# refresh-bio/kmer-db

Hardware: AMD Instinct MI355X
Metric: all2all k-mer pair-comparisons/sec (higher is better)
Workload: dtype u32

## Files before the change

### kmer-db_amd/csrc/a2a_blocks.hip

```cpp
#include "device_common.h"
#include "engine_internal.h"

#include "prim.h"

#include <algorithm>
#include <chrono>
#include <cmath>
#include <cstdio>
#include <cstdlib>
#include <cstring>
#include <functional>
#include <memory>
#include <string>

enum : uint32_t {
    KCTR_CHUNKS = 0,
    KCTR_POOL_OVERFLOW,
    KCTR_PAIR_OVERFLOW,
    KCTR_NWIDE,
    KCTR_LIST_OVERFLOW,
    KCTR_RAW = 5,
    KCTR_RECORDS = 6,
    KCTR_RECORDS_HI = 7,
    KCTR_SLOW = 8,
// ... 295 lines not shown
template <class PV> __device__ __forceinline__ void rowtab_finish(const RowTab& R, const PV& pv, uint32_t lane) {
    lds_sync();
    for (uint32_t X = lane; X < R.n; X += WAVE) {
        const uint32_t e = R.end[X];
        if (e) pool_cold(pv)->chunk_fill[(e - 1u) >> CH_SHIFT] = CH_REC - (e - R.pos[X]);
    }
}
template <bool ROWS, class PV>
__device__ __forceinline__ void rec_emit(WaveArena& A, const PV& pv, const RowTab& R, bool on, uint32_t X, unsigned long long rows, unsigned long long cols,
                                         uint32_t w, uint32_t stream, uint32_t lane, unsigned long long lt_mask) {
    if constexpr (ROWS) row_emit(A, pv, R, on, X, rows, cols, w, stream, lane, lt_mask);
    else wide_emit(A, pv, on, rows, cols, w, stream, lane, lt_mask);
}
__device__ __forceinline__ void rec_store_diag(const PoolView& pv, uint32_t slot, unsigned long long rows, uint32_t w) {
    const uint32_t ch = slot >> CH_SHIFT, r = slot & (CH_REC - 1u);
    ((unsigned long long*)(pv.rec + ((size_t)ch << (CH_SHIFT + 4))))[r] = rows;
    pv.recw[slot] = w;
}

__global__ void call_prologue_kernel(uint32_t* __restrict__ state, uint32_t n_state, uint32_t* __restrict__ chunk_fill, uint32_t* __restrict__ chunk_key,
                                     uint32_t pool_cap, unsigned char* __restrict__ touched, uint32_t n_touched) {
    const uint32_t i = blockIdx.x * blockDim.x + threadIdx.x;
    if (i < n_state) state[i] = 0u;
    if (i < pool_cap) { chunk_fill[i] = 0u; chunk_key[i] = 0xFFFFFFFFu; }
    if (i < n_touched) touched[i] = 0;
}

struct K0Params {
    const uint2* k0in;
    const uint32_t* bitrel;
    const uint64_t* blkbase;
    const uint64_t* bits;
    const uint32_t* perm;
    uint32_t P;
    uint32_t short_ids;
    BlockMap bm;
    unsigned long long* p0_mask;
    uint32_t* p0_info;
    uint32_t* pair_ofs;
    uint16_t* pair_blk;
    unsigned long long* pair_mask;
    uint32_t* pair_cursor;
    uint32_t n_regions, region_cap, spill_cap;
    uint32_t* counters;
};

constexpr int K0_RELW = 8;
constexpr int K0_SINGLE_PASS = 1;
template <bool LONG>
__global__ __launch_bounds__(256) void k0_decode_kernel(const K0Params q) {
    const uint32_t t = blockIdx.x * blockDim.x + threadIdx.x;
    const uint32_t lane = threadIdx.x & 63u;
    uint32_t i = 0;
    bool live;
    if (q.perm) {
        live = t < q.P;
        if (live) i = q.perm[t];
    } else {
        __shared__ uint32_t bins[64];
        __shared__ uint16_t order[256];
        if (threadIdx.x < 64) bins[threadIdx.x] = 0;
        __syncthreads();
        const uint2 kt = t < q.P ? q.k0in[t] : make_uint2(0u, 0u);
        const uint32_t tl = kmdb_k0_l(kt), tbits = kmdb_k0_bits(kt);
        uint32_t key = 0;
        if (t < q.P && tl > 1 && !kmdb_long_node(tl, tbits, q.short_ids)) {
            key = 1u + (tbits - (tl - 1u));
            key = key > 63u ? 63u : key;
        }
        atomicAdd(&bins[63u - key], 1u);
        __syncthreads();
        if (threadIdx.x < 64) {
            const uint32_t c = bins[threadIdx.x];
            bins[threadIdx.x] = wave_incl_scan(c, threadIdx.x) - c;
        }
        __syncthreads();
        order[atomicAdd(&bins[63u - key], 1u)] = (uint16_t)threadIdx.x;
        __syncthreads();
        i = blockIdx.x * blockDim.x + order[threadIdx.x];
        live = i < q.P;
    }
    const BlockMap bm = q.bm;
    const uint2 km = live ? q.k0in[i] : make_uint2(0u, 0u);
    const uint32_t l = kmdb_k0_l(km), last = kmdb_k0_last(km), nbits = kmdb_k0_bits(km);
    if (!q.perm && kmdb_long_node(l, nbits, q.short_ids)) live = false;
    using Cursor = RunCursor32<LONG ? 16 : 6, LONG>;
    uint32_t npairs = 0, blk0 = 0, need = 0, span = 0, bit0 = 0;
    unsigned long long mask0 = 0, m1 = 0, m2 = 0;
    bool second_pass = false, from_words = false;
    uint64_t pos = 0;
    unsigned long long rel_w[K0_RELW];
    uint32_t rel_i[K0_RELW], rel_n = 0;
#pragma unroll
    for (int e = 0; e < K0_RELW; ++e) { rel_w[e] = 0; rel_i[e] = 0; }
    auto rel_push = [&](uint32_t idx, unsigned long long w) {
#pragma unroll
        for (int e = 0; e < K0_RELW; ++e) if (rel_n == (uint32_t)e) { rel_w[e] = w; rel_i[e] = idx; }
        ++rel_n;
    };
    auto rel_blocks = [&](bool write, uint32_t id0, uint32_t o) -> uint32_t {
        const unsigned long long wm = bm.width == 64 ? ~0ull : (1ull << bm.width) - 1ull;
        uint32_t curblk = 0xFFFFFFFFu, cnt = 0;
        unsigned long long cacc = 0;
        auto flushb = [&]() {
            if (curblk == 0xFFFFFFFFu) return;
            if (write) { if (cnt == 0) mask0 = cacc; else { q.pair_blk[o] = (uint16_t)curblk; q.pair_mask[o] = cacc; ++o; } }
            ++cnt;
        };
#pragma unroll
        for (int e = 0; e < K0_RELW; ++e) {
            if ((uint32_t)e < rel_n) {
                const uint32_t base = id0 + 64u * rel_i[e];
                const unsigned long long word = rel_w[e];
                const uint32_t b = bm.blk(base);
                uint32_t bit = bm.bit(base, b), sh = 0;
#pragma unroll
                for (uint32_t part = 0; part < 3; ++part) {
                    if (sh < 64u) {
                        const unsigned long long m = ((word >> sh) << bit) & wm;
                        if (m) {
                            if (b + part != curblk) { flushb(); curblk = b + part; cacc = 0; }
                            cacc |= m;
                        }
                        sh += bm.width - bit; bit = 0;
                    }
                }
            }
        }
        flushb();
        return cnt;
    };
    if (live && l == 1) {
        blk0 = bm.blk(last); mask0 = 1ull << bm.bit(last, blk0); npairs = 1;
    } else if (live && l) {
        pos = q.blkbase[i >> 8] + q.bitrel[i];
        unsigned long long R = 1ull;
        {
            Cursor c(q.bits, pos);
            uint32_t rem = l - 1;
            uint32_t wk = 0;
            unsigned long long acc = 1ull;
            auto add = [&](uint32_t s0, uint32_t cnt) {
                while (cnt) {
                    const uint32_t k = s0 >> 6, o = s0 & 63u;
                    const uint32_t take = cnt < 64u - o ? cnt : 64u - o;
                    if (k != wk) { rel_push(wk, acc); wk = k; acc = 0; }
                    acc |= (take == 64u ? ~0ull : ((1ull << take) - 1ull)) << o;
                    s0 += take; cnt -= take;
                }
            };
            while (rem) {
                uint32_t z, v;
                c.step(rem, z, v);
                if (z) {
                    if (LONG) add(span + 1u, z);
                    else if (span + z < 64u) R |= ((2ull << (z - 1)) - 1ull) << (span + 1);
                    span += z; rem -= z;
                }
                if (v) {
                    span += v; --rem;
                    if (LONG) add(span, 1u);
                    else if (span < 64u) R |= 1ull << span;
                }
            }
            if (LONG) { if (span < 64u) R = acc; else rel_push(wk, acc); }
        }
        const uint32_t id0 = last - span;
        blk0 = bm.blk(id0);
        bit0 = bm.bit(id0, blk0);
        const unsigned long long wm = bm.width == 64 ? ~0ull : (1ull << bm.width) - 1ull;
// ... 2657 lines not shown
    const size_t W = node_cap / 64u, NB = b.NB;
    DEV_ALLOC(b.l2_cursors, 2 * L2_SUB * 16);
    DEV_ALLOC(b.l2_bitmap, NB * W);
    DEV_ALLOC(b.l2_rank, NB * W);
    DEV_ALLOC(b.l2_len, NB);
    DEV_ALLOC(b.l2_loff, NB + 2);
    DEV_ALLOC(b.l2_ent_g, (size_t)ent_cap);
    DEV_ALLOC(b.l2_ent_blk, (size_t)ent_cap);
    DEV_ALLOC(b.l2_ent_mask, (size_t)ent_cap);
    DEV_ALLOC(b.l2_list_mask, (size_t)ent_cap);
    DEV_ALLOC(b.l2_list_w, (size_t)ent_cap);
    DEV_ALLOC(b.l2_node_w, (size_t)node_cap);
    b.l2_node_cap = node_cap; b.l2_ent_cap = ent_cap;
    return 0;
}

struct Launched { uint32_t raw = 0, rowjobs = 0, k2jobs = 0; };
inline uint32_t with_slack(uint32_t v) { return v + v / 8u + 1024u; }
int stage_done(hipStream_t s, const char* name) {
    if (!kmdb_sync_debug()) return 0;
    const hipError_t e = hipStreamSynchronize(s);
    fprintf(stderr, "[kmdb] stage %-14s %s\n", name, e == hipSuccess ? "ok" : hipGetErrorString(e));
    return e == hipSuccess ? 0 : kmdb_set_error(std::string("stage ") + name + ": " + hipGetErrorString(e));
}
void a2a_prologue(BlocksState& b, hipStream_t st, bool decode) {
    const uint32_t pool_cap = (uint32_t)b.pool_cap;
    const uint32_t n_state = decode ? b.call_state_n_decode : b.call_state_n, n_touched = decode && b.tile_touched ? b.n_states + 1u : 0u;
    hipLaunchKernelGGL(call_prologue_kernel, dim3((std::max(std::max(n_state, pool_cap), n_touched) + 255u) / 256u), dim3(256), 0, st, b.call_state.get(), n_state,
                       b.chunk_fill.get(), b.chunk_key.get(), pool_cap, b.tile_touched.get(), n_touched);
}
int a2a_decode(kmdb_db* db, BlocksState& b, hipStream_t st) {
    const uint32_t P = (uint32_t)db->P;
    K0Params q{};
    q.k0in = db->k0in; q.bitrel = db->bitrel; q.blkbase = db->blkbase; q.bits = db->bits; q.perm = nullptr; q.P = P; q.short_ids = db->short_max_ids;
    q.bm = BlockMap{db->width, (uint32_t)((1ull << 32) / db->width) + 1u};
    q.p0_mask = b.p0_mask; q.p0_info = b.p0_info; q.pair_ofs = b.pair_ofs; q.pair_blk = b.pair_blk; q.pair_mask = b.pair_mask;
    uint32_t nreg = 1;
    while (nreg < KMDB_PAIR_REGIONS && (uint64_t)nreg * 16384 < P) nreg <<= 1;
    q.pair_cursor = b.pair_cursor; q.n_regions = nreg; q.region_cap = (uint32_t)(b.pair_cap * 3 / 4 / nreg);
    q.spill_cap = (uint32_t)(b.pair_cap - (uint64_t)q.region_cap * nreg); q.counters = b.counters;
    hipLaunchKernelGGL((k0_decode_kernel<false>), dim3((P + 255) / 256), dim3(256), 0, st, q);
    if (db->n_long) {
        q.perm = db->long_nodes; q.P = db->n_long;
        hipLaunchKernelGGL((k0_decode_kernel<true>), dim3((db->n_long + 255) / 256), dim3(256), 0, st, q);
    }
    HIP_TRY(hipGetLastError());
    return 0;
}
int a2a_narrow_emit(kmdb_db* db, BlocksState& b, uint32_t* M, uint32_t emit_lo, uint32_t emit_hi, hipStream_t st) {
    NParams q{};
    q.nl = db->nl; q.parent = db->parent; q.w = db->w; q.dflag = db->dflag; q.seg_anc = db->nseg_anc; q.seg_anc_n = db->nseg_anc_n;
    q.p0_mask = b.p0_mask; q.p0_info = b.p0_info; q.pair_ofs = b.pair_ofs; q.pair_blk = b.pair_blk; q.pair_mask = b.pair_mask;
    q.fn_mask = b.fn_mask; q.fn_blk = b.fn_blk; q.widebits = b.widebits; q.wide_base = b.wide_base; q.wide_slice_cnt = b.wide_slice_cnt;
    q.P = (uint32_t)db->P; q.nseg_nodes = db->nseg_nodes; q.n_segs = db->n_nsegs; q.chain_cap = db->chain_cap;
    q.emit_lo = emit_lo; q.emit_hi = emit_hi; q.tbits = b.dense_narrow ? 0u : arena_table_bits(b.g_rows); q.n_keys = b.g_rows;
    q.all_wide = b.dense_narrow ? 1u : 0u;
    q.pool = pool_view(b, b.dense_narrow);
    q.band_xlo = b.g_xlo; q.band_xhi = b.g_xhi; q.band_sbase = b.g_sbase;
    const size_t wave_lds = k1n_wave_bytes(q.chain_cap, q.tbits, q.n_keys, b.row_mode ? b.g_rows : 0u);
    const uint32_t waves = (uint32_t)std::max<size_t>(1, std::min<size_t>(K1N_WAVES, (144u << 10) / wave_lds));
    const size_t lds = wave_lds * waves;
    q.M = M; q.N = (uint32_t)db->N; q.bwidth = db->width; q.touched = touched_view(b); q.direct_ctr = b.direct_ctr;
    q.dmask = b.dmask; q.dwx = b.dwx; q.slice_cnt = b.slice_cnt;
    const K1nPick pick = b.emit_band ? k1n_band_pick(b.k1n_mode, b.row_mode) : k1n_pick(b.k1n_mode, b.knobs.k1n_minw, b.row_mode);
    HIP_TRY(hipFuncSetAttribute((const void*)pick.fn, hipFuncAttributeMaxDynamicSharedMemorySize, (int)lds));
    const dim3 grid((q.n_segs + waves - 1) / waves), block(WAVE * waves);
    if (!b.have_counts && kmdb_verbose())
        fprintf(stderr, "[kmdb] narrow kernel: %u slices, %zu B of LDS per wave, %u per workgroup, instantiation %s\n", q.n_segs, wave_lds, waves, pick.name);
    hipLaunchKernelGGL(pick.fn, grid, block, lds, st, q);
    HIP_TRY(hipGetLastError());
    return 0;
}
int a2a_slice_apply(kmdb_db* db, BlocksState& b, uint32_t* M, hipStream_t st, hipStream_t s2) {
    HIP_TRY(hipEventRecord(db->ev_side[0], st));
// ... 498 lines not shown
```

### kmer-db_amd/csrc/engine_state.h

```cpp
#pragma once
#include "kmdb_amd.h"
#include "kmdb_internal.h"

#include <thread>
#include "engine_internal.h"
#include "dev_mem.h"

#include <hip/hip_runtime.h>

#include <cstdint>
#include <memory>
#include <string>
#include <utility>
#include <vector>

struct Segment { uint32_t first, end; };

struct BlocksState;
struct BlocksStateDelete { void operator()(BlocksState* b) const; };

struct kmdb_db {
    int device = 0;
    uint64_t N = 0, P = 0;
    uint32_t kmer_length = 0;
    DevBuf<uint2> k0in;
    DevBuf<uint32_t> bitrel;
    DevBuf<uint64_t> blkbase;
    DevBuf<uint64_t> bits;
    uint64_t n_bit_words = 0;
    uint32_t short_max_ids = 48;
    DevBuf<uint32_t> nl;
    DevBuf<int32_t> parent;
    DevBuf<uint32_t> w;
    DevBuf<uint16_t> dflag;
    DevBuf<uint32_t> sub_end;
    DevBuf<uint32_t> long_nodes;
    uint32_t n_long = 0;
    uint32_t nseg_nodes = 2048;
    uint32_t n_nsegs = 0;
    DevBuf<uint32_t> nseg_anc;
    DevBuf<uint32_t> nseg_anc_n;
    uint32_t chain_cap = 8;
    uint32_t max_depth = 0, max_n = 0;
    DevBuf<unsigned long long> list_sets;
    uint32_t list_sets_nb = 0;
    bool list_sets_tried = false;
    DevBuf<uint32_t> rl_ofs;
    DevBuf<uint32_t> rl_runs;
    DevBuf<uint4> rl_node;
    bool rl_tried = false;
    bool chain_ok = false;
    uint32_t width = 64;
    std::unique_ptr<BlocksState, BlocksStateDelete> blocks;
    uint64_t blocks_bytes_counted = 0;
    bool last_call_sized = false;
    std::vector<std::pair<void*, size_t>> staging;
    std::vector<std::pair<void*, size_t>> staging_kept;
    std::thread staging_thread;
    bool one_shot = false;
    bool v1_ready = false;
    DevBuf<uint4> meta;
    DevBuf<uint64_t> bitpos;
    DevBuf<uint32_t> ck_ofs;
    DevBuf<uint64_t> ck_bit;
    DevBuf<uint32_t> ck_id;
    DevBuf<uint32_t> wprefix;
    DevBuf<Segment> segs;
    uint32_t n_segs = 0;
    DevBuf<void> v1_scan_tmp;
    size_t v1_scan_tmp_bytes = 0;
// ... 25 lines not shown
    uint64_t band_max_streams = 0;
    int band_emit_mode = -2;
    kmdb_all2all_rows_band_emit_stats be_stats{};
    uint64_t n_buckets = 0;
    DevBuf<uint64_t> bucket_offset;
    DevBuf<uint64_t> slots;
    DevBuf<uint32_t> pid2dfs;
    uint32_t qs_index = 0, qs_count = 0;
    hipStream_t stream = nullptr;
    hipStream_t stream2 = nullptr;
    DevEvent ev_side[2], ev[4];
    DevEvent ev_k[4];
    kmdb_stats stats{};
    kmdb_db2db_stats d2_stats{};
    kmdb_new2all_sparse_stats n2s_stats{};
    kmdb_sample_stats sample_stats{};
    kmdb_sample_stats d2_sample_stats{};
    kmdb_sample_stats n2a_sample_stats{};
    bool blocks_prepared = false;
    std::string fallback_reason;
};

constexpr uint32_t KMDB_MAX_STREAM_BITS = 1u << 24;
__host__ __device__ inline uint2 kmdb_k0_pack(uint32_t l, uint32_t last, uint32_t nbits) {
    uint2 r;
    r.x = l | ((nbits >> 12) << KMDB_ID_BITS); r.y = last | ((nbits & 0xFFFu) << KMDB_ID_BITS);
    return r;
}
__host__ __device__ inline uint32_t kmdb_k0_l(uint2 km) { return km.x & (KMDB_MAX_SAMPLES - 1u); }
__host__ __device__ inline uint32_t kmdb_k0_last(uint2 km) { return km.y & (KMDB_MAX_SAMPLES - 1u); }
__host__ __device__ inline uint32_t kmdb_k0_bits(uint2 km) { return ((km.x >> KMDB_ID_BITS) << 12) | (km.y >> KMDB_ID_BITS); }
constexpr uint32_t KMDB_SHORT_MAX_IDS = 48, KMDB_SHORT_MAX_BITS = 128;
__host__ __device__ inline bool kmdb_long_node(uint32_t l, uint32_t num_bits, uint32_t max_ids) { return l > max_ids || num_bits > KMDB_SHORT_MAX_BITS; }
constexpr int KMDB_CHAIN_MAX = 4096;

int kmdb_layout_upload(kmdb_db* db, const kmdb_db_view* v, int with_hashtables, const kmdb_kept_nodes* sel);
int kmdb_db_upload_planned(const kmdb_db_view* v, const kmdb_opts* opts, int with_hashtables, uint32_t shard_index, uint32_t shard_count, kmdb_shard_plan* plan,
                           kmdb_db** out);
int kmdb_db_upload_query_planned(const kmdb_db_view* v, const kmdb_opts* opts, uint32_t shard_index, uint32_t shard_count, kmdb_shard_plan* plan, kmdb_db** out);
int kmdb_db_upload_range_planned(const kmdb_db_view* v, const kmdb_opts* opts, uint32_t range_index, const kmdb_range_plan* plan, kmdb_db** out);

int kmdb_v1_run(kmdb_db* db, uint32_t* M, uint32_t seg_begin, uint32_t seg_end, uint32_t flags, hipStream_t st);

int kmdb_blocks_prepare(kmdb_db* db);
struct kmdb_band_desc { uint64_t row_lo, row_hi, cell_lo, cells; bool emit = false; };
int kmdb_blocks_run(kmdb_db* db, uint32_t* M, uint32_t emit_lo, uint32_t emit_hi, hipStream_t st, const kmdb_band_desc* band = nullptr);
std::string kmdb_blocks_band_refusal(const kmdb_db* db, const kmdb_band_geometry* g);
int kmdb_blocks_band_prepare(kmdb_db* db, const kmdb_band_geometry* g, uint64_t band_cells);
int kmdb_blocks_k1n_mode(const kmdb_db* db, bool band_state);
uint64_t kmdb_blocks_state_bytes(const kmdb_db* db, bool band_state);
struct kmdb_blocks_band_units { uint64_t jobs, jobs_run, runs, runs_run, slices, slices_run, tiles, tiles_run; };
struct kmdb_blocks_band_info { uint32_t key_bits, row_mode, l2_on, attempts, slices; uint64_t records, est_records; kmdb_blocks_band_units units; };
kmdb_blocks_band_info kmdb_blocks_band_last(const kmdb_db* db, bool band_state);
void kmdb_blocks_release(kmdb_db* db);
uint64_t kmdb_blocks_device_bytes(const kmdb_db* db);
int kmdb_blocks_ensure_prepared(kmdb_db* db);
int kmdb_blocks_stage_ms(kmdb_db* db, float ms[4]);
inline void kmdb_recount_bytes(kmdb_db* db, uint64_t& counted, uint64_t now) {
    db->stats.device_bytes = db->stats.device_bytes - counted + now;
    counted = now;
}
struct kmdb_blocks_counts { uint64_t records, direct; uint32_t wide, chunks, joined; };
kmdb_blocks_counts kmdb_blocks_last_counts(const kmdb_db* db);
const unsigned char* kmdb_blocks_tile_touched(const kmdb_db* db);
int kmdb_ensure_v1_arrays(kmdb_db* db);

// ... 2 lines not shown
```

### kmer-db_amd/csrc/kmdb_internal.h

```cpp
#pragma once
#include <cstddef>
#include <cstdint>
#include <functional>
#include <string>
#include <utility>
#include <vector>

int kmdb_set_error(const std::string& msg);

constexpr uint32_t KMDB_ABI_OLDEST_COMPATIBLE = 7, KMDB_ABI_THIS = 8;
inline bool kmdb_abi_compatible(uint32_t caller) { return caller >= KMDB_ABI_OLDEST_COMPATIBLE && caller <= KMDB_ABI_THIS; }

void kmdb_drop_pages(const std::vector<std::pair<void*, size_t>>& regions, unsigned threads);

struct kmdbh_db;
struct kmdbh_db_arrays {
    int64_t *num_kmers, *parent_id;
    uint32_t *num_samples, *num_local, *last_sample_id, *num_bits;
    uint64_t *data_offset, *data, *bucket_offset, *slots;
};
kmdbh_db* kmdbh_db_make(uint32_t kmer_length, double fraction, double start_fraction, int32_t alphabet, uint64_t kmers_count,
                        std::vector<std::string>&& names, std::vector<uint64_t>&& sample_kmers, uint64_t n_patterns, uint64_t n_data_words,
                        uint64_t n_buckets, uint64_t n_slots, kmdbh_db_arrays* arrays);

struct kmdb_db;
struct kmdb_layout_device_source {
    uint64_t n_patterns = 0, n_samples = 0;
    uint32_t kmer_length = 0;
    const long long* num_kmers = nullptr;
    const long long* parent_id = nullptr;
    const uint32_t* num_samples = nullptr;
    const uint32_t* num_local = nullptr;
    const uint32_t* last_sample_id = nullptr;
    const uint32_t* num_bits = nullptr;
    const unsigned long long* data_offset = nullptr;
    const uint64_t* data = nullptr;
    uint64_t n_data_words = 0;
    uint64_t n_buckets = 0, n_slots = 0;
    const uint64_t* bucket_offset = nullptr;
    const uint64_t* slots = nullptr;
    std::function<void()> tables_done, fields_done, streams_done;
    mutable double fields_ms = 0;
    double layout_ms = 0, prepare_ms = 0;
};
int kmdb_layout_from_device(kmdb_db* db, const kmdb_layout_device_source* src, int with_hashtables);
struct kmdb_opts;
int kmdb_db_from_device(kmdb_layout_device_source* src, const kmdb_opts* opts, int with_hashtables, kmdb_db** out);

using kmdb_device_lists_sink = std::function<int(const uint64_t* d_kmers, const uint64_t* off, size_t n, void* stream)>;
struct kmdb_opts;
int kmdb_minhash_device_lists(const char* who, const char* const* seqs, const size_t* seq_lens, size_t n_samples, uint32_t kmer_length, double fraction,
                              double start_fraction, int32_t alphabet, const kmdb_opts* opts, const kmdb_device_lists_sink& sink);

int kmdb_sorted_union_on_stream(const char* who, const uint64_t* a, uint64_t na, const uint64_t* b, uint64_t nb, uint64_t* out, uint64_t* n_out, void* stream,
                                uint64_t* scratch_bytes);

struct kmdb_db_view;
constexpr uint32_t KMDB_MAX_SHARDS = 4096;
struct kmdb_shard_plan {
    uint64_t P = 0;
    uint32_t n_shards = 0;
    std::vector<uint32_t*> w;
    std::vector<unsigned char*> mask;
    std::vector<uint64_t> kept;
    kmdb_shard_plan() = default;
    kmdb_shard_plan(const kmdb_shard_plan&) = delete;
    kmdb_shard_plan& operator=(const kmdb_shard_plan&) = delete;
    ~kmdb_shard_plan();
    void release_weights(uint32_t shard);
    bool keeps(uint32_t shard, uint64_t p) const { return (mask[shard >> 3][p] >> (shard & 7u)) & 1u; }
};
int kmdb_shard_plan_build(const kmdb_db_view* v, uint32_t n_shards, const std::vector<uint32_t>& shards, kmdb_shard_plan* plan);

void kmdb_query_shard_tables(const kmdb_db_view* v, uint32_t shard, uint32_t n_shards, uint64_t* n_buckets, uint64_t* n_slots);

template <class F>
inline void kmdb_for_bucket_runs(const uint64_t* kmers, size_t count, F&& fn) {
    for (size_t i = 0; i < count;) {
        const uint64_t b = kmers[i] >> 32;
        size_t e = i + 1;
// ... 44 lines not shown
```

### kmer-db_amd/csrc/layout.hip

```cpp
#include "device_common.h"
#include "engine_internal.h"

#include "prim.h"

#include <algorithm>
#include <atomic>
#include <chrono>
#include <cstdio>
#include <cstdlib>
#include <cstring>
#include <sys/mman.h>
#include <thread>

namespace {

struct U32toU64 { __host__ __device__ uint64_t operator()(uint32_t v) const { return v; } };

__global__ void lay_child_runs_kernel(const uint32_t* __restrict__ skeys, uint32_t P, uint32_t* __restrict__ start, uint32_t* __restrict__ cnt) {
    const uint32_t j = blockIdx.x * blockDim.x + threadIdx.x;
    if (j >= P) return;
    const uint32_t k = skeys[j];
    if (j == 0 || skeys[j - 1] != k) start[k] = j;
    if (j + 1 == P || skeys[j + 1] != k) cnt[k] = j + 1;
}
// ... 114 lines not shown
    if ((i & 255u) == 0) blkbase[i >> 8] = b;
    bitrel[i] = (uint32_t)(dstpos[i] - b);
}
__global__ void lay_copy_bits_kernel(const uint32_t* __restrict__ order, const uint64_t* __restrict__ srcpos, const uint64_t* __restrict__ dstpos,
                                     const uint2* __restrict__ k0in, const uint64_t* __restrict__ src, uint32_t P, unsigned long long* __restrict__ dst) {
    const uint32_t i = blockIdx.x * blockDim.x + threadIdx.x;
    if (i >= P) return;
    const uint32_t nb = kmdb_k0_bits(k0in[i]);
    if (!nb) return;
    uint64_t sp = srcpos[order[i]], dp = dstpos[i];
    for (uint32_t done = 0; done < nb; done += 64) {
        const uint32_t take = nb - done < 64u ? nb - done : 64u;
        const uint32_t ss = (uint32_t)(sp & 63u);
        uint64_t chunk = src[sp >> 6] << ss;
        if (ss && take > 64u - ss) chunk |= src[(sp >> 6) + 1] >> (64u - ss);
        if (take < 64u) chunk &= ~0ull << (64u - take);
        const uint32_t ds = (uint32_t)(dp & 63u);
        atomicOr(&dst[dp >> 6], (unsigned long long)(chunk >> ds));
        if (ds && take > 64u - ds) atomicOr(&dst[(dp >> 6) + 1], (unsigned long long)(chunk << (64u - ds)));
        sp += take; dp += take;
    }
}
struct LongNodePred {
    const uint2* k0in;
    uint32_t short_ids;
    __host__ __device__ bool operator()(uint32_t i) const { const uint2 km = k0in[i]; return kmdb_long_node(kmdb_k0_l(km), kmdb_k0_bits(km), short_ids); }
};
__global__ void lay_long_keys_kernel(const uint2* __restrict__ k0in, const uint32_t* __restrict__ idx, uint32_t n, uint32_t* __restrict__ keys) {
    const uint32_t t = blockIdx.x * blockDim.x + threadIdx.x;
    if (t >= n) return;
    const uint2 km = k0in[idx[t]];
    const uint32_t l = kmdb_k0_l(km);
    keys[t] = kmdb_k0_bits(km) - (l ? l - 1u : 0u);
}
__global__ void lay_seg_anc_kernel(const int32_t* __restrict__ parent, const uint16_t* __restrict__ dflag, uint32_t P, uint32_t nseg_nodes, uint32_t n_segs,
                                   uint32_t chain_cap, uint32_t* __restrict__ anc, uint32_t* __restrict__ anc_n) {
    const uint32_t s = blockIdx.x * blockDim.x + threadIdx.x;
    if (s >= n_segs) return;
    int32_t cur = parent[(size_t)s * nseg_nodes];
    uint32_t d = cur < 0 ? 0u : (uint32_t)(dflag[cur] & 0x7FFFu);
    if (d > chain_cap) d = 0;
    anc_n[s] = d;
    while (cur >= 0 && d) { anc[(size_t)s * chain_cap + (--d)] = (uint32_t)cur; cur = parent[cur]; }
}

struct HostRegion { void* p; size_t bytes; };
template <class T>
struct HostBuf {
    T* p = nullptr;
    size_t bytes = 0;
    explicit HostBuf(size_t n, bool zero = false) {
        (void)zero;
        bytes = (std::max<size_t>(n, 1) * sizeof(T) + 4095) & ~(size_t)4095;
        void* q = mmap(nullptr, bytes, PROT_READ | PROT_WRITE, MAP_PRIVATE | MAP_ANONYMOUS, -1, 0);
        p = q == MAP_FAILED ? nullptr : (T*)q;
    }
    ~HostBuf() { reset(); }
    void reset() { if (p) (void)munmap(p, bytes); p = nullptr; }
    HostRegion release() { HostRegion r{p, bytes}; p = nullptr; return r; }
    T& operator[](size_t i) { return p[i]; }
    HostBuf(const HostBuf&) = delete;
    HostBuf& operator=(const HostBuf&) = delete;
};

struct LayPhase {
    const bool verbose = getenv("KMDB_VERBOSE") != nullptr;
// ... 413 lines not shown
    if (in.streams_done) in.streams_done();
    phase("device: stream re-pack");

    db->max_n = hs.max_n; db->max_depth = hs.max_depth;
    db->chain_ok = hs.max_depth <= (uint32_t)KMDB_CHAIN_MAX;
    db->chain_cap = std::min<uint32_t>(KMDB_CHAIN_MAX, std::max<uint32_t>(8, (hs.max_depth + 7) / 8 * 8));
    db->nseg_nodes = 2048;
    if (const char* e = getenv("KMDB_NSEG")) if (*e) db->nseg_nodes = (uint32_t)std::max<uint64_t>(64, strtoull(e, nullptr, 10) / 64 * 64);
    db->n_nsegs = (uint32_t)((P + db->nseg_nodes - 1) / db->nseg_nodes);
    DEV_ALLOC(db->nseg_anc, std::max<size_t>((size_t)db->n_nsegs * db->chain_cap, 1));
    DEV_ALLOC(db->nseg_anc_n, std::max<size_t>(db->n_nsegs, 1));
    if (db->n_nsegs)
        hipLaunchKernelGGL(lay_seg_anc_kernel, dim3((db->n_nsegs + 63) / 64), dim3(64), 0, st, db->parent, db->dflag, (uint32_t)P, db->nseg_nodes, db->n_nsegs,
                           db->chain_cap, db->nseg_anc, db->nseg_anc_n);
    db->n_long = hs.n_long;
    if (hs.n_long) {
        DevBuf<uint32_t> sel, lk, lk2, nsel;
        if (sel.alloc(hs.n_long + 1) || lk.alloc(std::max<size_t>(hs.n_long, 1)) || lk2.alloc(std::max<size_t>(hs.n_long, 1)) || nsel.alloc(1)) return 1;
        DEV_ALLOC(db->long_nodes, (size_t)hs.n_long);
        rocprim::counting_iterator<uint32_t> first(0u);
        size_t tb = 0;
        HIP_TRY(prim::select_if(nullptr, tb, first, sel.get(), nsel.get(), (int)P, LongNodePred{db->k0in, db->short_max_ids}, st));
        DevBuf<unsigned char> tmp;
        if (tmp.alloc(std::max<size_t>(tb, 1))) return 1;
        HIP_TRY(prim::select_if(tmp.get(), tb, first, sel.get(), nsel.get(), (int)P, LongNodePred{db->k0in, db->short_max_ids}, st));
        hipLaunchKernelGGL(lay_long_keys_kernel, dim3((hs.n_long + 255) / 256), dim3(256), 0, st, db->k0in, sel.get(), hs.n_long, lk.get());
        size_t tb2 = 0;
        HIP_TRY(prim::sort_pairs_desc(nullptr, tb2, lk.get(), lk2.get(), sel.get(), db->long_nodes.get(), (int)hs.n_long, 0, 32, st));
        DevBuf<unsigned char> tmp2;
        if (tmp2.alloc(std::max<size_t>(tb2, 1))) return 1;
        HIP_TRY(prim::sort_pairs_desc(tmp2.get(), tb2, lk.get(), lk2.get(), sel.get(), db->long_nodes.get(), (int)hs.n_long, 0, 32, st));
        HIP_TRY(hipStreamSynchronize(st));
    }
    HIP_TRY(hipStreamSynchronize(st));
    phase("device: slices + long nodes");

    db->stats.algorithmic_bytes = hs.alg + 4ull * (N ? N * (N - 1) / 2 : 0);
    db->stats.tree_updates = hs.upd;
    db->stats.sum_pairs = hs.pairs;
    db->stats.n_segments = db->n_nsegs;
    db->stats.n_patterns = P;
    db->stats.h2d_bytes = in.h2d_bytes;
    db->stats.device_bytes = P * (8 + 4 + 4 + 4 + 4 + 2 + 4) + n_bit_words * 8 + (uint64_t)db->n_nsegs * db->chain_cap * 4 + in.dev_ht_bytes;
    return 0;
}
}

int kmdb_layout_from_device(kmdb_db* db, const kmdb_layout_device_source* s, int with_hashtables) {
    const uint64_t P = s->n_patterns, N = s->n_samples;
    const auto t0 = std::chrono::steady_clock::now();
    LayPhase phase;
    hipStream_t st = db->stream;
    LayIn in;
    in.P = P; in.N = N;
    DevBuf<unsigned long long> total;
    DevBuf<uint32_t> bad;
    if (in.parent.alloc(P) || in.ll.alloc(P) || in.last.alloc(P) || in.n.alloc(P) || in.nbits.alloc(P) || in.w.alloc(P) || in.wfull.alloc(P) || in.srcpos.alloc(P + 1) ||
        total.alloc(1) || bad.alloc(2)) return 1;
    HIP_TRY(hipMemsetAsync(total.get(), 0, 8, st));
    HIP_TRY(hipMemsetAsync(bad.get(), 0, 8, st));
    hipLaunchKernelGGL(lay_fields_kernel, dim3((unsigned)((P + 255) / 256)), dim3(256), 0, st, s->num_kmers, s->parent_id, s->num_samples, s->num_local, s->last_sample_id,
                       s->num_bits, s->data_offset, s->n_data_words, (uint32_t)P, (uint32_t)N, in.parent.get(), in.ll.get(), in.last.get(), in.n.get(), in.nbits.get(), in.w.get(),
                       in.wfull.get(), in.srcpos.get(), total.get(), bad.get());
    HIP_TRY(hipGetLastError());
    unsigned long long total_bits = 0;
    uint32_t hbad[2] = {0, 0};
    HIP_TRY(hipMemcpyAsync(&total_bits, total.get(), 8, hipMemcpyDeviceToHost, st));
    HIP_TRY(hipMemcpyAsync(hbad, bad.get(), 8, hipMemcpyDeviceToHost, st));
    HIP_TRY(hipStreamSynchronize(st));
    if (hbad[0]) return kmdb_set_error("kmdb_db_upload: parent_id >= pattern id");
    if (hbad[1]) return kmdb_set_error("kmdb_db_upload: inconsistent pattern header");
    if (s->fields_done) s->fields_done();
    in.n_bit_words = (total_bits + 63) / 64 + 16;
    in.src = s->data;
    if (with_hashtables && s->n_buckets) {
        db->n_buckets = s->n_buckets;
        DEV_ALLOC(db->bucket_offset, s->n_buckets + 1);
        DEV_ALLOC(db->slots, std::max<uint64_t>(s->n_slots, 1));
// ... 13 lines not shown
```

Before: 20300 billion.

## Precompute per-window k0 decode order and skip bitstream reads for run-only nodes

Moves the per-block bin sort of short nodes out of the decode kernel into a one-time layout kernel that writes a per-window order and live count. The decode kernel reads that precomputed order and returns early for waves with no live items. Nodes whose encoding is a single contiguous run are decoded directly from l without touching the bit stream. This cuts per-call sorting, shared-memory syncs and wasted waves, at the cost of extra device memory and a layout-time pass.

```diff
diff --git a/kmer-db_amd/csrc/a2a_blocks.hip b/kmer-db_amd/csrc/a2a_blocks.hip
--- a/kmer-db_amd/csrc/a2a_blocks.hip
+++ b/kmer-db_amd/csrc/a2a_blocks.hip
@@ -351,8 +351,11 @@
     const uint64_t* blkbase;
     const uint64_t* bits;
     const uint32_t* perm;
+    const uint16_t* order;
+    const uint32_t* live;
+    uint32_t win_shift;
+    uint32_t n_items;
     uint32_t P;
-    uint32_t short_ids;
     BlockMap bm;
     unsigned long long* p0_mask;
     uint32_t* p0_info;
@@ -368,41 +371,27 @@
 constexpr int K0_SINGLE_PASS = 1;
 template <bool LONG>
 __global__ __launch_bounds__(256) void k0_decode_kernel(const K0Params q) {
-    const uint32_t t = blockIdx.x * blockDim.x + threadIdx.x;
     const uint32_t lane = threadIdx.x & 63u;
     uint32_t i = 0;
     bool live;
-    if (q.perm) {
+    if constexpr (LONG) {
+        const uint32_t t = blockIdx.x * blockDim.x + threadIdx.x;
         live = t < q.P;
         if (live) i = q.perm[t];
     } else {
-        __shared__ uint32_t bins[64];
-        __shared__ uint16_t order[256];
-        if (threadIdx.x < 64) bins[threadIdx.x] = 0;
-        __syncthreads();
-        const uint2 kt = t < q.P ? q.k0in[t] : make_uint2(0u, 0u);
-        const uint32_t tl = kmdb_k0_l(kt), tbits = kmdb_k0_bits(kt);
-        uint32_t key = 0;
-        if (t < q.P && tl > 1 && !kmdb_long_node(tl, tbits, q.short_ids)) {
-            key = 1u + (tbits - (tl - 1u));
-            key = key > 63u ? 63u : key;
-        }
-        atomicAdd(&bins[63u - key], 1u);
-        __syncthreads();
-        if (threadIdx.x < 64) {
-            const uint32_t c = bins[threadIdx.x];
-            bins[threadIdx.x] = wave_incl_scan(c, threadIdx.x) - c;
-        }
-        __syncthreads();
-        order[atomicAdd(&bins[63u - key], 1u)] = (uint16_t)threadIdx.x;
-        __syncthreads();
-        i = blockIdx.x * blockDim.x + order[threadIdx.x];
-        live = i < q.P;
+        const uint32_t sub_shift = q.win_shift - 8u;
+        const uint32_t k = blockIdx.x >> 3;
+        const uint32_t w = sub_shift ? ((k >> sub_shift) << 3) + (blockIdx.x & 7u) : blockIdx.x;
+        if ((w << sub_shift) >= q.n_items) return;
+        const uint32_t r = ((k & ((1u << sub_shift) - 1u)) << 8) + threadIdx.x;
+        const uint32_t n_live = q.live[w];
+        if ((r & ~63u) >= n_live) return;
+        live = r < n_live;
+        if (live) i = (w << q.win_shift) + q.order[((size_t)w << q.win_shift) + r];
     }
     const BlockMap bm = q.bm;
     const uint2 km = live ? q.k0in[i] : make_uint2(0u, 0u);
     const uint32_t l = kmdb_k0_l(km), last = kmdb_k0_last(km), nbits = kmdb_k0_bits(km);
-    if (!q.perm && kmdb_long_node(l, nbits, q.short_ids)) live = false;
     using Cursor = RunCursor32<LONG ? 16 : 6, LONG>;
     uint32_t npairs = 0, blk0 = 0, need = 0, span = 0, bit0 = 0;
     unsigned long long mask0 = 0, m1 = 0, m2 = 0;
@@ -452,9 +441,12 @@
     if (live && l == 1) {
         blk0 = bm.blk(last); mask0 = 1ull << bm.bit(last, blk0); npairs = 1;
     } else if (live && l) {
-        pos = q.blkbase[i >> 8] + q.bitrel[i];
         unsigned long long R = 1ull;
-        {
+        if (!LONG && kmdb_k0_run_only(l, nbits)) {
+            R = (2ull << (l - 1u)) - 1ull;
+            span = l - 1u;
+        } else {
+            pos = q.blkbase[i >> 8] + q.bitrel[i];
             Cursor c(q.bits, pos);
             uint32_t rem = l - 1;
             uint32_t wk = 0;
@@ -3178,14 +3170,20 @@
 int a2a_decode(kmdb_db* db, BlocksState& b, hipStream_t st) {
     const uint32_t P = (uint32_t)db->P;
     K0Params q{};
-    q.k0in = db->k0in; q.bitrel = db->bitrel; q.blkbase = db->blkbase; q.bits = db->bits; q.perm = nullptr; q.P = P; q.short_ids = db->short_max_ids;
+    q.k0in = db->k0in; q.bitrel = db->bitrel; q.blkbase = db->blkbase; q.bits = db->bits; q.perm = nullptr; q.P = P;
     q.bm = BlockMap{db->width, (uint32_t)((1ull << 32) / db->width) + 1u};
     q.p0_mask = b.p0_mask; q.p0_info = b.p0_info; q.pair_ofs = b.pair_ofs; q.pair_blk = b.pair_blk; q.pair_mask = b.pair_mask;
     uint32_t nreg = 1;
     while (nreg < KMDB_PAIR_REGIONS && (uint64_t)nreg * 16384 < P) nreg <<= 1;
     q.pair_cursor = b.pair_cursor; q.n_regions = nreg; q.region_cap = (uint32_t)(b.pair_cap * 3 / 4 / nreg);
     q.spill_cap = (uint32_t)(b.pair_cap - (uint64_t)q.region_cap * nreg); q.counters = b.counters;
-    hipLaunchKernelGGL((k0_decode_kernel<false>), dim3((P + 255) / 256), dim3(256), 0, st, q);
+    q.order = db->k0_order; q.live = db->k0_live;
+    q.win_shift = 8;
+    while ((1u << q.win_shift) < db->k0_window) ++q.win_shift;
+    const uint32_t wgs_per_win = db->k0_window >> 8;
+    q.n_items = (uint32_t)((db->P + db->k0_window - 1) / db->k0_window) * wgs_per_win;
+    const uint32_t grid = wgs_per_win > 1 ? (q.n_items + 8u * wgs_per_win - 1u) / (8u * wgs_per_win) * (8u * wgs_per_win) : q.n_items;
+    if (grid) hipLaunchKernelGGL((k0_decode_kernel<false>), dim3(grid), dim3(256), 0, st, q);
     if (db->n_long) {
         q.perm = db->long_nodes; q.P = db->n_long;
         hipLaunchKernelGGL((k0_decode_kernel<true>), dim3((db->n_long + 255) / 256), dim3(256), 0, st, q);
diff --git a/kmer-db_amd/csrc/engine_state.h b/kmer-db_amd/csrc/engine_state.h
--- a/kmer-db_amd/csrc/engine_state.h
+++ b/kmer-db_amd/csrc/engine_state.h
@@ -36,6 +36,9 @@
     DevBuf<uint32_t> sub_end;
     DevBuf<uint32_t> long_nodes;
     uint32_t n_long = 0;
+    DevBuf<uint16_t> k0_order;
+    DevBuf<uint32_t> k0_live;
+    uint32_t k0_window = 256;
     uint32_t nseg_nodes = 2048;
     uint32_t n_nsegs = 0;
     DevBuf<uint32_t> nseg_anc;
@@ -127,6 +130,15 @@
 __host__ __device__ inline uint32_t kmdb_k0_bits(uint2 km) { return ((km.x >> KMDB_ID_BITS) << 12) | (km.y >> KMDB_ID_BITS); }
 constexpr uint32_t KMDB_SHORT_MAX_IDS = 48, KMDB_SHORT_MAX_BITS = 128;
 __host__ __device__ inline bool kmdb_long_node(uint32_t l, uint32_t num_bits, uint32_t max_ids) { return l > max_ids || num_bits > KMDB_SHORT_MAX_BITS; }
+__host__ __device__ inline bool kmdb_k0_run_only(uint32_t l, uint32_t num_bits) { return l > 1 && num_bits <= l - 1u; }
+__host__ __device__ inline uint32_t kmdb_k0_key(uint32_t l, uint32_t num_bits, uint32_t max_ids) {
+    if (kmdb_long_node(l, num_bits, max_ids)) return 0u;
+    if (l <= 1) return 1u;
+    if (kmdb_k0_run_only(l, num_bits)) return 2u;
+    const uint32_t extra = num_bits - (l - 1u);
+    return extra > 61u ? 63u : 2u + extra;
+}
+constexpr uint32_t KMDB_K0_WINDOW_MIN = 256, KMDB_K0_WINDOW_MAX = 4096, KMDB_K0_WINDOW_DEFAULT = 256;
 constexpr int KMDB_CHAIN_MAX = 4096;
 
 int kmdb_layout_upload(kmdb_db* db, const kmdb_db_view* v, int with_hashtables, const kmdb_kept_nodes* sel);
diff --git a/kmer-db_amd/csrc/kmdb_internal.h b/kmer-db_amd/csrc/kmdb_internal.h
--- a/kmer-db_amd/csrc/kmdb_internal.h
+++ b/kmer-db_amd/csrc/kmdb_internal.h
@@ -46,6 +46,7 @@
 int kmdb_layout_from_device(kmdb_db* db, const kmdb_layout_device_source* src, int with_hashtables);
 struct kmdb_opts;
 int kmdb_db_from_device(kmdb_layout_device_source* src, const kmdb_opts* opts, int with_hashtables, kmdb_db** out);
+extern "C" int kmdb_debug_k0_order(const kmdb_db* db, uint32_t* window, uint64_t* n_windows, uint16_t* order, uint32_t* live, uint32_t* l, uint32_t* num_bits);
 
 using kmdb_device_lists_sink = std::function<int(const uint64_t* d_kmers, const uint64_t* off, size_t n, void* stream)>;
 struct kmdb_opts;
diff --git a/kmer-db_amd/csrc/layout.hip b/kmer-db_amd/csrc/layout.hip
--- a/kmer-db_amd/csrc/layout.hip
+++ b/kmer-db_amd/csrc/layout.hip
@@ -170,6 +170,28 @@
     const uint2 km = k0in[idx[t]];
     const uint32_t l = kmdb_k0_l(km);
     keys[t] = kmdb_k0_bits(km) - (l ? l - 1u : 0u);
+}
+__global__ __launch_bounds__(256) void lay_k0_order_kernel(const uint2* __restrict__ k0in, uint32_t P, uint32_t W, uint32_t short_ids, uint16_t* __restrict__ order,
+                                                           uint32_t* __restrict__ live) {
+    __shared__ uint32_t bins[64];
+    const uint64_t base = (uint64_t)blockIdx.x * W;
+    auto key_of = [&](uint32_t r) -> uint32_t {
+        if (base + r >= P) return 0u;
+        const uint2 km = k0in[base + r];
+        return kmdb_k0_key(kmdb_k0_l(km), kmdb_k0_bits(km), short_ids);
+    };
+    if (threadIdx.x < 64) bins[threadIdx.x] = 0;
+    __syncthreads();
+    for (uint32_t r = threadIdx.x; r < W; r += 256) atomicAdd(&bins[63u - key_of(r)], 1u);
+    __syncthreads();
+    if (threadIdx.x < 64) {
+        const uint32_t c = bins[threadIdx.x];
+        const uint32_t first = wave_incl_scan(c, threadIdx.x) - c;
+        bins[threadIdx.x] = first;
+        if (threadIdx.x == 63) live[blockIdx.x] = first;
+    }
+    __syncthreads();
+    for (uint32_t r = threadIdx.x; r < W; r += 256) order[base + atomicAdd(&bins[63u - key_of(r)], 1u)] = (uint16_t)r;
 }
 __global__ void lay_seg_anc_kernel(const int32_t* __restrict__ parent, const uint16_t* __restrict__ dflag, uint32_t P, uint32_t nseg_nodes, uint32_t n_segs,
                                    uint32_t chain_cap, uint32_t* __restrict__ anc, uint32_t* __restrict__ anc_n) {
@@ -649,8 +671,23 @@
         HIP_TRY(prim::sort_pairs_desc(tmp2.get(), tb2, lk.get(), lk2.get(), sel.get(), db->long_nodes.get(), (int)hs.n_long, 0, 32, st));
         HIP_TRY(hipStreamSynchronize(st));
     }
+    db->k0_window = KMDB_K0_WINDOW_DEFAULT;
+    if (const char* e = getenv("KMDB_K0_WINDOW")) if (*e) {
+        const uint32_t want = (uint32_t)std::max(0, atoi(e));
+        uint32_t w = KMDB_K0_WINDOW_MIN;
+        while (w < KMDB_K0_WINDOW_MAX && w < want) w <<= 1;
+        db->k0_window = w;
+    }
+    const uint64_t n_windows = (P + db->k0_window - 1) / db->k0_window;
+    DEV_ALLOC(db->k0_order, std::max<uint64_t>(n_windows * db->k0_window, 1));
+    DEV_ALLOC(db->k0_live, std::max<uint64_t>(n_windows, 1));
+    if (n_windows) {
+        hipLaunchKernelGGL(lay_k0_order_kernel, dim3((unsigned)n_windows), dim3(256), 0, st, db->k0in, (uint32_t)P, db->k0_window, db->short_max_ids,
+                           db->k0_order.get(), db->k0_live.get());
+        HIP_TRY(hipGetLastError());
+    }
     HIP_TRY(hipStreamSynchronize(st));
-    phase("device: slices + long nodes");
+    phase("device: slices + long nodes + decode order");
 
     db->stats.algorithmic_bytes = hs.alg + 4ull * (N ? N * (N - 1) / 2 : 0);
     db->stats.tree_updates = hs.upd;
@@ -658,9 +695,30 @@
     db->stats.n_segments = db->n_nsegs;
     db->stats.n_patterns = P;
     db->stats.h2d_bytes = in.h2d_bytes;
-    db->stats.device_bytes = P * (8 + 4 + 4 + 4 + 4 + 2 + 4) + n_bit_words * 8 + (uint64_t)db->n_nsegs * db->chain_cap * 4 + in.dev_ht_bytes;
+    db->stats.device_bytes = P * (8 + 4 + 4 + 4 + 4 + 2 + 4) + n_bit_words * 8 + (uint64_t)db->n_nsegs * db->chain_cap * 4 + in.dev_ht_bytes +
+                             n_windows * db->k0_window * 2 + n_windows * 4;
     return 0;
 }
+}
+
+extern "C" int kmdb_debug_k0_order(const kmdb_db* db, uint32_t* window, uint64_t* n_windows, uint16_t* order, uint32_t* live, uint32_t* l, uint32_t* num_bits) {
+    if (!db) return kmdb_set_error("kmdb_debug_k0_order: null handle");
+    const uint64_t nw = (db->P + db->k0_window - 1) / db->k0_window;
+    if (window) *window = db->k0_window;
+    if (n_windows) *n_windows = nw;
+    HIP_TRY(hipSetDevice(db->device));
+    HIP_TRY(hipStreamSynchronize(db->stream));
+    if (order && nw) HIP_TRY(hipMemcpy(order, db->k0_order.get(), nw * db->k0_window * 2, hipMemcpyDeviceToHost));
+    if (live && nw) HIP_TRY(hipMemcpy(live, db->k0_live.get(), nw * 4, hipMemcpyDeviceToHost));
+    if ((l || num_bits) && db->P) {
+        std::vector<uint2> km(db->P);
+        HIP_TRY(hipMemcpy(km.data(), db->k0in.get(), db->P * sizeof(uint2), hipMemcpyDeviceToHost));
+        for (uint64_t i = 0; i < db->P; ++i) {
+            if (l) l[i] = kmdb_k0_l(km[i]);
+            if (num_bits) num_bits[i] = kmdb_k0_bits(km[i]);
+        }
+    }
+    return 0;
 }
 
 int kmdb_layout_from_device(kmdb_db* db, const kmdb_layout_device_source* s, int with_hashtables) {
diff --git a/profiles/decode_order_census.py b/profiles/decode_order_census.py
--- /dev/null
+++ b/profiles/decode_order_census.py
@@ -0,0 +1,215 @@
+#!/usr/bin/env python3
+import json
+import os
+import sys
+
+import numpy as np
+import torch
+
+ROOT = os.path.dirname(os.path.dirname(os.path.abspath(__file__)))
+sys.path.insert(0, ROOT)
+SEED = 20260929
+SHORT_IDS, SHORT_BITS = 48, 128
+
+
+def dfs_index(parent):
+    P = parent.numel()
+    dev = parent.device
+    ar = torch.arange(P, device=dev)
+
+    def along_paths(val):
+        val, anc = val.clone(), parent.clone()
+        while True:
+            m = anc >= 0
+            if not bool(m.any()):
+                return val
+            a = anc[m]
+            val[m] += val[a]
+            anc[m] = anc[a]
+    depth = along_paths(torch.ones(P, dtype=torch.int64, device=dev))
+    size = torch.ones(P, dtype=torch.int64, device=dev)
+    by_depth = torch.argsort(depth, stable=True)
+    counts = torch.bincount(depth)
+    ends = torch.cumsum(counts, 0).tolist()
+    for level in range(int(depth.max()), 1, -1):
+        nodes = by_depth[ends[level - 1]: ends[level]]
+        size.index_add_(0, parent[nodes], size[nodes])
+    fam = torch.argsort(parent, stable=True)
+    csum = torch.cumsum(size[fam], 0) - size[fam]
+    fp = parent[fam]
+    first = torch.ones(P, dtype=torch.bool, device=dev)
+    first[1:] = fp[1:] != fp[:-1]
+    start = torch.cummax(torch.where(first, torch.arange(P, device=dev), torch.zeros((), dtype=torch.int64, device=dev)), 0)[0]
+    rel = torch.empty(P, dtype=torch.int64, device=dev)
+    rel[fam] = csum - csum[start] + (fp >= 0).to(torch.int64)
+    del ar
+    return along_paths(rel)
+
+
+def decode_steps(nl, nb, doff, data):
+    dev = nl.device
+    u = np.ascontiguousarray(data.view(np.uint32).reshape(-1, 2)[:, ::-1]).reshape(-1).astype(np.int64)
+    U = torch.from_numpy(np.concatenate([u, np.zeros(2, np.int64)])).to(dev)
+    idx = torch.nonzero(nl > 1).squeeze(1)
+    pos0 = doff[idx] * 64
+    pos, left = pos0.clone(), nl[idx] - 1
+    steps = torch.zeros(nl.numel(), dtype=torch.int64, device=dev)
+    zero_behind = torch.zeros(nl.numel(), dtype=torch.bool, device=dev)
+    bad = 0
+    while idx.numel():
+        k, s = pos >> 5, pos & 31
+        v = (((U[k] << 32) | U[k + 1]) >> (32 - s)) & 0xFFFFFFFF
+        inv = (~v) & 0xFFFFFFFF
+        assert bool((inv > 0).all()), "a code of 32 ones or more"
+        ones = 32 - torch.frexp(inv.double())[1].to(torch.int64)
+        pos = pos + 2 * ones + 1
+        steps[idx] += (ones > 0).to(torch.int64)
+        zero_behind[idx] = ones == 0
+        left = left - 1
+        done = left == 0
+        if bool(done.any()):
+            bad += int((pos[done] - pos0[done] != nb[idx[done]]).sum())
+            keep = ~done
+            idx, pos, pos0, left = idx[keep], pos[keep], pos0[keep], left[keep]
+    assert bad == 0, "%d streams do not end where num_bits says" % bad
+    return steps + zero_behind.to(torch.int64)
+
+
+def keys_of(nl, nb):
+    long_ = (nl > SHORT_IDS) | (nb > SHORT_BITS)
+    extra = nb - (nl - 1)
+    key = torch.clamp(2 + extra, max=63)
+    key = torch.where(extra == 0, torch.full_like(key, 2), key)
+    key = torch.where(nl == 1, torch.ones_like(key), key)
+    return torch.where(long_ | (nl == 0), torch.zeros_like(key), key), long_
+
+
+def wave_iterations(key, steps, W):
+    P = key.numel()
+    pad = (-P) % W
+    k = torch.cat([key, torch.zeros(pad, dtype=key.dtype, device=key.device)])
+    s = torch.cat([steps, torch.zeros(pad, dtype=steps.dtype, device=key.device)])
+    win = torch.arange(k.numel(), device=key.device) // W
+    order = torch.argsort(win * 64 + (63 - k), stable=True)
+    return float(s[order].view(-1, 64).max(dim=1)[0].sum()) * 256.0 / P
+
+
+def census(arr, dev):
+    t = lambda a: torch.from_numpy(np.ascontiguousarray(a.astype(np.int64))).to(dev)
+    parent, nl, nb, doff = t(arr["parent_id"]), t(arr["num_local"]), t(arr["num_bits"]), t(arr["data_offset"])
+    P = nl.numel()
+    pre = dfs_index(parent)
+    assert bool((torch.sort(pre)[0] == torch.arange(P, device=dev)).all()), "the pre-order is a permutation"
+    steps_pid = decode_steps(nl, nb, doff, arr["data"])
+    inv = torch.empty_like(pre)
+    inv[pre] = torch.arange(P, device=dev)
+    nl, nb, steps = nl[inv], nb[inv], steps_pid[inv]
+    key, long_ = keys_of(nl, nb)
+    run_only = (nl > 1) & (nb == nl - 1) & ~long_
+    short = key > 0
+    steps = torch.where(short, steps, torch.zeros_like(steps))
+    after = torch.where(run_only, torch.zeros_like(steps), steps)
+    coded = short & ~run_only & (nl > 1)
+    hist = torch.bincount(torch.clamp(steps[coded], max=32), minlength=33).tolist()
+    out = {"patterns": P, "share_l1": float((nl == 1).sum()) / P, "share_run_only": float(run_only.sum()) / P, "share_long": float(long_.sum()) / P,
+           "share_empty": float((nl == 0).sum()) / P, "mean_steps_short": float(steps[short].sum()) / max(int(short.sum()), 1),
+           "mean_steps_coded": float(steps[coded].sum()) / max(int(coded.sum()), 1), "steps_hist_coded_0_to_32plus": hist,
+           "wave_iterations_per_256": {"before_256": wave_iterations(key, steps, 256)}}
+    for W in (256, 1024, 4096):
+        out["wave_iterations_per_256"]["after_%d" % W] = wave_iterations(key, after, W)
+    out["wave_iterations_per_256"]["after_ideal"] = float(after.sum()) / 64.0 * 256.0 / P
+    live_waves = {}
+    for W in (256, 1024, 4096):
+        pad = (-P) % W
+        k = torch.cat([key, torch.zeros(pad, dtype=key.dtype, device=dev)]).view(-1, W)
+        n_live, n_coded = (k > 0).sum(1), (k > 2).sum(1)
+        live_waves[str(W)] = {"live": float(((n_live + 63) // 64).sum()) * 256.0 / P, "reading_a_stream": float(((n_coded + 63) // 64).sum()) * 256.0 / P}
+    out["waves_per_256"] = live_waves
+    return out
+
+
+def generator_stamp():
+    import hashlib
+    h = hashlib.sha256()
+    for fn in (os.path.join(ROOT, "kmer-db_amd", "synth.py"), os.path.join(ROOT, "bench.py")):
+        with open(fn, "rb") as f:
+            h.update(f.read())
+    return h.hexdigest()[:16]
+
+
+def arrays_of(name, fresh=False):
+    import shutil
+    import bench as B
+    wl = B.WORKLOADS[name]
+    cache = "/dev/shm/kmdb_ab_%s_n%d_c%d_l%d_k18_seed%d" % (name, wl["samples"], wl["clade_size"], wl["length"], SEED)
+    stamp_file, stamp = os.path.join(cache, "generator_sha16"), generator_stamp()
+    if os.path.exists(os.path.join(cache, "done")):
+        if not fresh and os.path.exists(stamp_file) and open(stamp_file).read().strip() == stamp:
+            return {nm[:-4]: np.load(os.path.join(cache, nm)) for nm in os.listdir(cache) if nm.endswith(".npy")}, "cache %s (generator %s)" % (cache, stamp)
+        shutil.rmtree(cache)
+    arr = B.generate_in_child(0, n_samples=wl["samples"], clade_size=wl["clade_size"], length=wl["length"], k=18, seed=SEED, rank=0, world=1)[0]
+    os.makedirs(cache, exist_ok=True)
+    for nm, a in arr.items():
+        np.save(os.path.join(cache, nm + ".npy"), a)
+    with open(stamp_file, "w") as f:
+        f.write(stamp + "\n")
+    open(os.path.join(cache, "done"), "w").close()
+    return arr, "generated (generator %s)" % stamp
+
+
+def selftest():
+    sys.path.insert(0, os.path.join(ROOT, "tests"))
+    from _kmerdb_loader import import_kmerdb_amd
+    import_kmerdb_amd()
+    import importlib
+    S = importlib.import_module("kmerdb_amd.synth")
+    g, pat = S.synth_database(60, 7, 3000, k=18, seed=5, device="cpu")
+    arr = S.to_view_arrays(pat)
+    parent = arr["parent_id"]
+    P = parent.size
+    kids = [[] for _ in range(P)]
+    roots = []
+    for p in range(P):
+        (kids[parent[p]] if parent[p] >= 0 else roots).append(p)
+    pre, stack, n = np.zeros(P, np.int64), roots[::-1], 0
+    while stack:
+        p = stack.pop()
+        pre[p] = n
+        n += 1
+        stack.extend(kids[p][::-1])
+    t = lambda a: torch.from_numpy(np.ascontiguousarray(a.astype(np.int64)))
+    assert np.array_equal(dfs_index(t(parent)).numpy(), pre), "DFS order"
+    lp, ids = pat["local_ptr"].numpy(), pat["local_ids"].numpy()
+    want = np.zeros(P, np.int64)
+    for p in range(P):
+        d = np.diff(ids[lp[p]: lp[p + 1]])
+        want[p] = int((d > 1).sum()) + int(d.size > 0 and d[-1] == 1)
+    got = decode_steps(t(arr["num_local"]), t(arr["num_bits"]), t(arr["data_offset"]), arr["data"]).numpy()
+    assert np.array_equal(got, want), "steps"
+    c = census(arr, torch.device("cpu"))
+    print("selftest ok:", json.dumps(c))
+
+
+def main():
+    if sys.argv[1:] == ["--selftest"]:
+        return selftest()
+    dev = torch.device("cuda", 0)
+    path = os.path.join(ROOT, "profiles", "decode_order_census.json")
+    out = {}
+    if os.path.exists(path):
+        with open(path) as f:
+            out = json.load(f)
+    fresh = "--fresh" in sys.argv
+    for name in [a for a in sys.argv[1:] if a != "--fresh"]:
+        arr, source = arrays_of(name, fresh)
+        out[name] = dict(census(arr, dev), arrays=source)
+        print("CENSUS %s %s" % (name, json.dumps(out[name])), flush=True)
+        torch.cuda.empty_cache()
+    dst = os.environ.get("CENSUS_OUT", path)
+    with open(dst, "w") as f:
+        json.dump(out, f, indent=1)
+        f.write("\n")
+
+
+if __name__ == "__main__":
+    main()
```

Measured after the change: 20820 billion (median of 6 runs). 2.6% higher.
